# ArnauGabrielAtienza/pytorch_distributed_examples

Hardware: AMD Instinct MI355X
Metric: images/sec (whole node) MNIST DDP + ResNet50 RPC-MP at 1/2/4/8 MI355X (higher is better)
Workload: dtype bf16; 1 GPU; model=mnist_cnn_Net, global_batch=1024, image=1x28x28, parallelism=dp1, hipgraph=True, fused_step=True, rccl_nranks=1, steps_per_graph=5, allreduce=none

## Files before the change

csrc/kernels/cnn_fused.hip:

```cpp
#include <cstddef>
#include <type_traits>

#include "adasum_weights.h"
#include "common.cuh"
#include "optim_device.h"
#include "pde_kernels.h"
#include "xgmi_device.h"

namespace pde {

namespace {

constexpr int T = 1024;
constexpr int NW = T / 64;
constexpr int NI = 4;
constexpr int C1 = 10, C2 = 20, KS = 5, H0 = 28, O1 = 24, P1 = 12, O2 = 8, P2 = 4, F1 = 50, F2 = 10;
constexpr int NX = H0 * H0, NC1 = P1 * P1, NR1 = C1 * NC1, NC2 = P2 * P2, NIN = C2 * NC2;
constexpr int RP16 = 146, RP8 = 148;
static_assert(RP16 >= NC1 && RP8 >= NC1, "channel planes hold the 144 cells");
static_assert(RP16 % 2 == 0 && RP8 % 4 == 0, "P9 reads 4 cells' argmax bytes as one aligned 4-byte word");
constexpr int EP = 148;
constexpr unsigned char AM_DEAD = 0xFF;
constexpr int XP = 36, NXP = H0 * XP;
constexpr int DHP = 52;
constexpr int W1N = C1 * KS * KS, W2N = C2 * C1 * KS * KS, FC1N = F1 * NIN, FC2N = F2 * F1;
constexpr int K2 = C1 * KS * KS;
constexpr int C1P = 16;
constexpr int KS2 = (KS * KS * C1P + 31) / 32;
constexpr int KSW2 = NI * 8 * 8 / 32;
constexpr int CG = 3;
constexpr int NGD = KS * KS * CG;
constexpr int KSD = (NGD + 3) / 4;
constexpr int D2N_P = 24, D2N_RP = 264, D2N_Q = 128;
constexpr int D2N_IM = 7 * D2N_RP + 7 * D2N_P + 2 * D2N_Q + 8;
static_assert(D2N_IM % 8 == 0 && D2N_P % 8 == 0 && D2N_RP % 8 == 0 && D2N_Q % 8 == 0, "d2n: 16-byte slots");
__host__ __device__ constexpr int d2n_ofs(int im, int y, int x, int co) {
  return im * D2N_IM + y * D2N_RP + x * D2N_P + (co >> 3) * D2N_Q + (co & 7);
}
constexpr int D2R = O2 * O2 + 8;
constexpr int MT1 = O1 * O1 / 16;
constexpr int MTD = NC1 * 1 / 16;
constexpr int KSW1 = O1 * O1 / 32;
struct KsRange {
  int lo, hi;
};
__host__ __device__ constexpr bool p7b_tap_live(int cls, int r, int ky, int kx) {
  const int pos = cls * 16 + r, y = pos / P1 - ky, x = pos % P1 - kx;
  return y >= 0 && y < O2 && x >= 0 && x < O2;
}
__host__ __device__ constexpr KsRange p7b_ks_range(int cls) {
  int lo = KSD, hi = 0;
  for (int r = 0; r < 16; ++r)
    for (int ky = 0; ky < KS; ++ky)
      for (int kx = 0; kx < KS; ++kx) {
        if (!p7b_tap_live(cls, r, ky, kx)) continue;
        const int g0 = (ky * KS + kx) * CG, k0 = g0 / 4, k1 = (g0 + CG - 1) / 4;
        lo = k0 < lo ? k0 : lo;
        hi = k1 + 1 > hi ? k1 + 1 : hi;
      }
  return {lo, hi};
}
__host__ __device__ constexpr bool p7b_range_covers(int cls, KsRange q) {
  for (int g = 0; g < NGD; ++g)
    for (int r = 0; r < 16; ++r)
      if (p7b_tap_live(cls, r, g / CG / KS, g / CG % KS) && (g / 4 < q.lo || g / 4 >= q.hi)) return false;
  return q.lo >= 0 && q.hi <= KSD;
}
__host__ __device__ constexpr bool p7b_ranges_ok() {
  int sum = 0;
  for (int c = 0; c < MTD; ++c) {
    if (!p7b_range_covers(c, p7b_ks_range(c))) return false;
    sum += p7b_ks_range(c).hi - p7b_ks_range(c).lo;
  }
  return sum == 126;
}
constexpr bool ks_is(KsRange q, int lo, int hi) { return q.lo == lo && q.hi == hi; }
static_assert(MTD == 9 && NC1 % 16 == 0 && p7b_ranges_ok(), "conv2 dgrad: every live tap inside its class's range");
static_assert(ks_is(p7b_ks_range(0), 0, 7) && ks_is(p7b_ks_range(1), 0, 12) && ks_is(p7b_ks_range(2), 0, 15) &&
                  ks_is(p7b_ks_range(3), 0, KSD) && ks_is(p7b_ks_range(4), 0, KSD) &&
                  ks_is(p7b_ks_range(5), 0, KSD) && ks_is(p7b_ks_range(6), 3, KSD) &&
                  ks_is(p7b_ks_range(7), 7, KSD) && ks_is(p7b_ks_range(8), 12, KSD),
              "conv2 dgrad k-step ranges (rows 0-1, 1-2, 2-3, 4..7, 8-9, 9-10, 10-11)");
__host__ __device__ constexpr uint64_t p7b_pack(bool hi) {
  uint64_t v = 0;
  for (int c = 0; c < MTD; ++c)
    v |= static_cast<uint64_t>(hi ? p7b_ks_range(c).hi : p7b_ks_range(c).lo) << (5 * c);
  return v;
}
constexpr uint64_t P7B_LO = p7b_pack(false), P7B_HI = p7b_pack(true);
static_assert(KSD < 32 && MTD * 5 <= 64, "5-bit fields");
constexpr int P7B_WCLS[NW] = {3, 4, 5, 5, 3, 4, 6, 6, 1, 7, 2, 2, 1, 7, 0, 0};
constexpr int P7B_WPAIR[NW] = {0, 0, 0, 1, 1, 1, 0, 1, 0, 0, 0, 1, 1, 1, 0, 1};
__host__ __device__ constexpr int p7b_wave_steps(int w) {
  const int c = P7B_WCLS[w];
  int n = p7b_ks_range(c).hi - p7b_ks_range(c).lo;
  if (c == 0) n += p7b_ks_range(MTD - 1).hi - p7b_ks_range(MTD - 1).lo;
  return 2 * n;
}
__host__ __device__ constexpr bool p7b_map_ok() {
  for (int c = 0; c < MTD - 1; ++c) {
    int n[2] = {0, 0};
    for (int w = 0; w < NW; ++w)
      if (P7B_WCLS[w] == c) ++n[P7B_WPAIR[w]];
    if (n[0] != 1 || n[1] != 1) return false;
  }
  int tot = 0;
  for (int s = 0; s < 4; ++s) {
    int n = 0;
    for (int w = s; w < NW; w += 4) n += p7b_wave_steps(w);
    if (n < 120 || n > 132) return false;
    tot += n;
  }
  return tot == NI * 126;
}
static_assert(NW == 16 && NI == 4 && p7b_map_ok(), "conv2 dgrad wave map: complete, balanced over the SIMDs");
__host__ __device__ constexpr uint64_t p7b_pack_map(bool pair) {
  uint64_t v = 0;
  for (int w = 0; w < NW; ++w) v |= static_cast<uint64_t>(pair ? P7B_WPAIR[w] : P7B_WCLS[w]) << (4 * w);
  return v;
}
constexpr uint64_t P7B_MCLS = p7b_pack_map(false), P7B_MPAIR = p7b_pack_map(true);
constexpr int O_W1 = 0, O_B1 = O_W1 + W1N, O_W2 = O_B1 + C1, O_B2 = O_W2 + W2N, O_FC1W = O_B2 + C2,
              O_FC1B = O_FC1W + FC1N, O_FC2W = O_FC1B + F1, O_FC2B = O_FC2W + FC2N, NPARAM = O_FC2B + F2;
constexpr int NSLAB = NPARAM - FC1N;
static_assert(O_W2 % 4 == 0 && C2 % 4 == 0 && W2N % 4 == 0, "W2T: float4 columns of 4 co");
constexpr int SLAB_OFS = (32 - O_W2 % 32) % 32;
constexpr int NSLABP = (SLAB_OFS + NSLAB + 31) / 32 * 32;
constexpr int S_FC1B = O_FC1B - FC1N, S_FC2W = O_FC2W - FC1N, S_FC2B = O_FC2B - FC1N;
constexpr int NACT = F1 + NIN;
__host__ __device__ constexpr int act_pitch(int nwg) { return (nwg * NI + 7) & ~7; }
static_assert(O_FC1W % 4 == 0 && FC1N % 4 == 0 && NSLAB % 4 == 0, "float4 slab columns");

__device__ __forceinline__ float hash_u01(unsigned long long seed, unsigned long long id) {
  unsigned long long z = seed + 0x9E3779B97F4A7C15ULL * (id + 1);
  z = (z ^ (z >> 30)) * 0xBF58476D1CE4E5B9ULL;
  z = (z ^ (z >> 27)) * 0x94D049BB133111EBULL;
  z ^= z >> 31;
  return static_cast<float>(z >> 40) * (1.0f / 16777216.0f);
}

__device__ __forceinline__ f32x4 mfma(const u16x8& a, const u16x8& b, const f32x4& c) {
  return __builtin_amdgcn_mfma_f32_16x16x32_bf16(__builtin_bit_cast(bf16x8, a), __builtin_bit_cast(bf16x8, b), c, 0,
                                                 0, 0);
}

template <int CTRL>
__device__ __forceinline__ float dppf(float v) {
  return __builtin_bit_cast(float, __builtin_amdgcn_update_dpp(0, __builtin_bit_cast(int, v), CTRL, 0xF, 0xF, false));
}
__device__ __forceinline__ float lanef(float v, int l) {
  return __builtin_bit_cast(float, __builtin_amdgcn_readlane(__builtin_bit_cast(int, v), l));
}
constexpr int DPP_XOR1 = 0xB1, DPP_XOR2 = 0x4E, DPP_HALF_MIRROR = 0x141, DPP_MIRROR = 0x140;
template <class Op>
__device__ __forceinline__ float wave_all(float v, Op op) {
  v = op(v, dppf<DPP_XOR1>(v));
  v = op(v, dppf<DPP_XOR2>(v));
  v = op(v, dppf<DPP_HALF_MIRROR>(v));
  v = op(v, dppf<DPP_MIRROR>(v));
  return op(op(lanef(v, 0), lanef(v, 16)), op(lanef(v, 32), lanef(v, 48)));
}
__device__ __forceinline__ float wave_sum_dpp(float v) { return wave_all(v, [](float a, float b) { return a + b; }); }
__device__ __forceinline__ float wave_max_dpp(float v) { return wave_all(v, [](float a, float b) { return fmaxf(a, b); }); }

struct CnnSmem {
  alignas(16) uint16_t r1n[NI][NC1][C1P];
  alignas(16) u16x8 w2f[KS2][2][64];
  alignas(16) u16x8 w2d[KSD][64];
  alignas(16) u16x8 w1f[64];
  alignas(16) uint16_t d2n[NI * D2N_IM];
  alignas(16) uint16_t d2[NI][C2][D2R];
  alignas(16) uint16_t zero16[8];
  alignas(8) uint32_t p7tab[KSD * 4][2];
  uint16_t x[NI][NXP];
  uint16_t xpad[18];
  uint16_t x1[NI][NXP];
  uint16_t xonepad[48];
  alignas(16) uint16_t xone[NI][NXP];
  alignas(16) uint16_t r1[NI][C1 * RP16];
  alignas(16) float b1[C1];
  alignas(16) float b2[C2];
  alignas(16) float fc1b[F1];
  alignas(16) float fc2w[FC2N];
  alignas(16) float fc2b[F2];
  alignas(16) float r2[NI][NIN];
  alignas(16) float dp2[NI][NIN];
  float h1[NI][F1], m1[NI][F1], h1d[NI][F1];
  alignas(16) float dh[NI][DHP];
  float mc2[NI][C2];
  float logit[NI][F2], dlog[NI][F2];
  float lossim[NI];
  float valid[NI];
  int label[NI];
  alignas(16) unsigned char a1[NI][C1 * RP8];
  unsigned char a2[NI][NIN];
};
static_assert(sizeof(CnnSmem) <= 160 * 1024, "LDS budget");
static_assert((offsetof(CnnSmem, xone) - offsetof(CnnSmem, x)) / 4 % 32 == 4,
              "xone bank offset from x (P9 B reads: scripts/p9_lds_model.py; x1's: cnn_p1)");
static_assert(offsetof(CnnSmem, w2f) == offsetof(CnnSmem, r1n) + sizeof(uint16_t) * NI * NC1 * C1P &&
                  sizeof(uint32_t) * NI * C1 * EP <= sizeof(uint16_t) * NI * NC1 * C1P + sizeof(u16x8) * KS2 * 2 * 64,
              "e1 aliases r1n + w2f");
static_assert(offsetof(CnnSmem, d2n) == offsetof(CnnSmem, w1f) + sizeof(u16x8) * 64 &&
                  NW * 2 * 64 * sizeof(f32x4) <= sizeof(u16x8) * (KSD * 64 + 64) + sizeof(uint16_t) * NI * D2N_IM,
              "P9 partials alias w2d + w1f + d2n (not e1)");
static_assert(offsetof(CnnSmem, w2d) == offsetof(CnnSmem, w2f) + sizeof(u16x8) * KS2 * 2 * 64, "w2f, w2d adjacent");
constexpr int NT2 = 16 / NW;
constexpr int NFRAG = KS2 * 2 * 64 + KSD * 64 + 64;
constexpr int NF2F = KS2 * 2 * 64, NF2D = KSD * 64;
static_assert(NF2F <= 2 * T && NF2D <= 2 * T && NF2F + NF2D + 64 == NFRAG, "fragment slots");
static_assert(offsetof(CnnSmem, w1f) == offsetof(CnnSmem, w2d) + sizeof(u16x8) * KSD * 64, "w2d, w1f adjacent");
constexpr int FC1_KC = NIN / 32;
constexpr int DP2_JC = 3;
constexpr int DP2_J = 16;
static_assert(F1 - DP2_J * (DP2_JC - 1) <= 20 && DP2_J % 4 == 0 && DHP >= DP2_J * (DP2_JC - 1) + 20, "dp2 chunks");
static_assert(F1 * FC1_KC <= T && NIN * DP2_JC <= T, "fc1 work split");
static_assert(sizeof(float) * NI * NIN * DP2_JC <= sizeof(u16x8) * KS2 * 2 * 64, "dp2 partials alias w2f");
static_assert(NT2 * NW == 16, "conv2 wgrad tiling");

__device__ __forceinline__ void lds_sync() {
  __builtin_amdgcn_fence(__ATOMIC_RELEASE, "workgroup", "local");
  __builtin_amdgcn_s_barrier();
  __builtin_amdgcn_fence(__ATOMIC_ACQUIRE, "workgroup", "local");
}

__device__ __forceinline__ uint32_t lds_addr(const void* p) {
#if defined(__HIP_DEVICE_COMPILE__)
  return (uint32_t)(const __attribute__((address_space(3))) unsigned char*)(p);
#else
  return static_cast<uint32_t>(reinterpret_cast<uintptr_t>(p));
#endif
}
__device__ __forceinline__ u16x8 lds_read16(uint32_t o) {
#if defined(__HIP_DEVICE_COMPILE__)
  return *(const __attribute__((address_space(3))) u16x8*)(o);
#else
  return u16x8{static_cast<uint16_t>(o), 0, 0, 0, 0, 0, 0, 0};
#endif
}

__device__ __forceinline__ void out_st(float* p, float v) {
  asm volatile("global_store_dword %0, %1, off sc1" ::"v"(p), "v"(v) : "memory");
}
__device__ __forceinline__ void out_st_u16x4(uint16_t* p, u16x4 v) { st_vec(reinterpret_cast<u16x4*>(p), v, true); }
__device__ __forceinline__ void out_st4(float* p, f32x4 v) {
  asm volatile("global_store_dwordx4 %0, %1, off sc1" ::"v"(p), "v"(v) : "memory");
}

template <bool TRAIN, class Smem>
__device__ __forceinline__ void cnn_p0(Smem& S, int t, int n0, int B, const float* __restrict__ images,
                                       const int64_t* __restrict__ tgt, const float* __restrict__ params,
                                       const u16x8* __restrict__ frag, const unsigned long long* __restrict__ rng,
                                       float p_drop2, float p_drop1, int training, u16x8 (&fr)[2]) {
  static_assert(NI * NX / 4 <= T, "one image quad per thread");
  constexpr int NH = C1 + C2 + F1 + FC2N + F2;
  static_assert(NH <= T && O_FC2W == O_FC1B + F1 && O_FC2B == O_FC2W + FC2N, "fc1b, fc2w, fc2b contiguous");
  static_assert(offsetof(Smem, fc2b) == offsetof(Smem, fc2w) + sizeof(float) * FC2N, "fc2w, fc2b adjacent");
  static_assert((NI & (NI - 1)) == 0 && 384 % NI == 0, "label threads 384..: slot t & (NI - 1)");
  const int qi = min(t, NI * NX / 4 - 1);
  const int qim = (qi * 4) / NX, qoff = qi * 4 - qim * NX;
  const int hi = min(t, NH - 1);
  const int hsrc = hi < C1 ? O_B1 + hi : hi < C1 + C2 ? O_B2 + hi - C1 : O_FC1B + hi - (C1 + C2);
  const int lslot = t & (NI - 1);
  const int64_t* lbase = tgt != nullptr ? tgt : reinterpret_cast<const int64_t*>(frag);
  const int lidx = tgt != nullptr ? min(n0 + lslot, B - 1) : 0;
  int rofs = 0;
  asm("" : "+v"(rofs));
  const u16x8 fw1 = frag[NF2F + NF2D + (t & 63)];
  const f32x4 img = *reinterpret_cast<const f32x4*>(images + static_cast<long>(min(n0 + qim, B - 1)) * NX + qoff);
  const float hv = params[hsrc];
  unsigned long long r0 = 0;
  if constexpr (TRAIN) r0 = rng[rofs];
  const int lab = reinterpret_cast<const int*>(lbase)[2 * lidx];
  fr[0] = frag[t];
  fr[1] = frag[min(t + T, NF2F - 1)];
  static_assert(H0 % 4 == 0 && XP >= H0 + 6, "image quads within a row; kx = 5 reads stay in the row");
  for (int i = t; i < NI * H0 * (XP - H0 + 1); i += T) {
    const int r = i / (XP - H0 + 1), c = i - r * (XP - H0 + 1);
    if (c > 0) (&S.x[0][0])[r * XP + H0 - 1 + c] = 0;
    (&S.x1[0][0])[r * XP + H0 - 1 + c] = 0;
  }
  if constexpr (TRAIN) {
    constexpr int NZ = (sizeof(Smem::d2n) + sizeof(Smem::d2)) / 16;
    static_assert(offsetof(Smem, d2) == offsetof(Smem, d2n) + sizeof(Smem::d2n) && sizeof(Smem::d2n) % 16 == 0 &&
                      sizeof(Smem::d2) % 16 == 0 && NZ > T && NZ <= 2 * T,
                  "d2n, d2 adjacent: two 16-byte stores per thread");
    static_assert(sizeof(Smem::d2n) == sizeof(uint16_t) * NI * D2N_IM &&
                      d2n_ofs(NI - 1, O2 - 1, O2 - 1, CG * 8 - 1) == NI * D2N_IM - 1 && d2n_ofs(0, 0, 0, 0) == 0,
                  "d2n: the zeroed extent is first to last slot of (image, y, x, co < 24)");
    {
      u16x8* z = reinterpret_cast<u16x8*>(&S.d2n[0]);
      z[t] = u16x8{0, 0, 0, 0, 0, 0, 0, 0};
      if (t + T < NZ) z[t + T] = u16x8{0, 0, 0, 0, 0, 0, 0, 0};
    }
    if (t < 8) S.zero16[t] = 0;
    static_assert((NI * NXP) % 8 == 0 && NI * NXP / 8 <= T, "xone: one 16-byte store per thread");
    if (t < NI * NXP / 8)
      reinterpret_cast<u16x8*>(&S.xone[0][0])[t] =
          u16x8{0x3F80, 0x3F80, 0x3F80, 0x3F80, 0x3F80, 0x3F80, 0x3F80, 0x3F80};
    if (t < KSD * 4) {
      const int g = t, tap = g / CG, cg = g - tap * CG, ky = tap / KS, kx = tap - ky * KS;
      S.p7tab[g][0] = g < NGD ? (static_cast<uint32_t>(ky) << 16) | static_cast<uint32_t>(kx) : 0x80008000u;
      S.p7tab[g][1] = static_cast<uint32_t>(g < NGD ? (-(ky * D2N_RP + kx * D2N_P) + cg * D2N_Q) * 2 : 0);
    }
  }
  if (t < 64) S.w1f[t] = fw1;
  if (t < NI * NX / 4) {
    const int im = qim, off = qoff, n = n0 + im;
    const f32x4 v = n < B ? img : f32x4{0.f, 0.f, 0.f, 0.f};
    const int row = off / H0, col = off - row * H0;
    uint16_t* dst = &S.x[im][row * XP + col];
    const uint16_t b0 = f2bf(v[0]), b1 = f2bf(v[1]), b2 = f2bf(v[2]), b3 = f2bf(v[3]);
    dst[0] = b0; dst[1] = b1; dst[2] = b2; dst[3] = b3;
    uint16_t* d1 = &S.x1[im][row * XP + col];
    if (col > 0) d1[-1] = b0;
    d1[0] = b1; d1[1] = b2; d1[2] = b3;
  }
  if (t < NH) {
    const int hofs = hi < C1             ? static_cast<int>(offsetof(Smem, b1)) + 4 * hi
                     : hi < C1 + C2      ? static_cast<int>(offsetof(Smem, b2)) + 4 * (hi - C1)
                     : hi < C1 + C2 + F1 ? static_cast<int>(offsetof(Smem, fc1b)) + 4 * (hi - (C1 + C2))
                                         : static_cast<int>(offsetof(Smem, fc2w)) + 4 * (hi - (C1 + C2 + F1));
    *reinterpret_cast<float*>(reinterpret_cast<unsigned char*>(&S) + hofs) = hv;
  }
  if constexpr (TRAIN) {
    const unsigned long long seed = r0 * 0xD1B54A32D192ED03ULL;
    const float keep2 = training ? 1.f / (1.f - p_drop2) : 1.f;
    const float keep1 = training ? 1.f / (1.f - p_drop1) : 1.f;
    if (t < NI * C2) {
      const int im = t / C2, c = t - im * C2;
      const unsigned long long id = static_cast<unsigned long long>(n0 + im) * C2 + c;
      S.mc2[im][c] = (!training || hash_u01(seed ^ 0x5bd1e995ULL, id) >= p_drop2) ? keep2 : 0.f;
    } else if (t >= 128 && t < 128 + NI * F1) {
      const int u = t - 128, im = u / F1, j = u - im * F1;
      const unsigned long long id = static_cast<unsigned long long>(n0 + im) * F1 + j;
      S.m1[im][j] = (!training || hash_u01(seed ^ 0x27d4eb2fULL, id) >= p_drop1) ? keep1 : 0.f;
    }
  }
  if (t >= 384 && t < 384 + NI) {
    const bool ok = tgt != nullptr && n0 + lslot < B;
    if constexpr (TRAIN) S.valid[lslot] = ok ? 1.f : 0.f;
    S.label[lslot] = ok ? static_cast<int>(lab) : 0;
  }
}


__device__ __forceinline__ float pool4(const f32x4& v, int& am) {
  am = 0;
  float m = v[0];
  if (v[1] > m) { m = v[1]; am = 1; }
  if (v[2] > m) { m = v[2]; am = 2; }
  if (v[3] > m) { m = v[3]; am = 3; }
  return m;
}

static_assert(P1 % 4 == 0 && MT1 * 4 == NC1, "conv1 tiles: 4 cells of one row");
static_assert((NI * MT1) % NW == 0, "every wave runs the same number of conv1 tiles");
constexpr int NT1 = NI * MT1 / NW;
constexpr int P1_TR = P1 / 4;
static_assert(MT1 % NT1 == 0, "conv1: a wave's tiles lie in one image");
static_assert(NT1 % P1_TR == 0, "conv1: a wave's tiles are whole cell rows");
constexpr int P1_WI = MT1 / NT1;
constexpr int P1_WR = NT1 / P1_TR;
struct P1Tile {
  int im, py, px0;
};
__host__ __device__ constexpr P1Tile p1_tile(int w, int u) {
  return {w / P1_WI, (w % P1_WI) * P1_WR + u / P1_TR, (u % P1_TR) * 4};
}
__host__ __device__ constexpr bool p1_map_ok() {
  for (int tile = 0; tile < NI * MT1; ++tile) {
// ... 243 lines not shown
    fd[1] = frag[NF2F + min(iw + TW, NF2D - 1)];
  }
  constexpr int JPER = F1 - DP2_J * (DP2_JC - 1);
  float w6[JPER];
  {
    const int tc = min(t, NIN * DP2_JC - 1);
    const int jc = tc / NIN, i = tc - jc * NIN;
#pragma unroll
    for (int u = 0; u < JPER; ++u) w6[u] = gFC1W[min(jc * DP2_J + u, F1 - 1) * NIN + i];
  }

  static_assert(NI <= NW, "P4: a wave per image");
  if (wid < NI) {
    const int im = wid, v = lane >> 2, p = lane & 3;
    const bool lv = v < F2;
    const auto [logit, lse, ly, y] = cnn_head(S, S.h1d[im], im, lane);
    const float val = S.valid[im];
    const float dl = (__expf(logit - lse) - (v == y ? 1.f : 0.f)) * val;
    if (lv && p == 0) S.dlog[im][v] = dl;
    if (lane == 0) S.lossim[im] = val * (lse - ly);
    static_assert(F1 <= 64, "P4: a lane per fc1 output");
    const int j = lane < F1 ? lane : 0;
    float sh = 0.f;
#pragma unroll
    for (int vv = 0; vv < F2; ++vv) sh += S.fc2w[vv * F1 + j] * lanef(dl, 4 * vv);
    if (lane < F1) S.dh[im][lane] = (S.h1[im][lane] > 0.f) ? sh * S.m1[im][lane] : 0.f;
  } else {
    static_assert(NC1 % 2 == 0 && RP16 % 2 == 0 && C1 > 8 && C1 <= 10 && C1P == 16 && NI * NC1 <= TW,
                  "r1 from r1n: cell pairs as aligned words, channels 0..7 | 8, 9");
    if (iw < NI * NC1) {
      const uint32_t uw = static_cast<uint32_t>(iw);
      const uint32_t im = uw / NC1, cp = (uw - im * NC1) >> 1, h = uw & 1;
      const uint32_t* src = reinterpret_cast<const uint32_t*>(&S.r1n[0][0][0]) + (uw >> 1) * C1P + h * 4;
      const u32x4 ev = *reinterpret_cast<const u32x4*>(src), od = *reinterpret_cast<const u32x4*>(src + C1P / 2);
      uint32_t* dst = reinterpret_cast<uint32_t*>(&S.r1[im][0]) + h * 8 * (RP16 / 2) + cp;
#pragma unroll
      for (int d = 0; d < 4; ++d)
        if (d == 0 || h == 0) {
          dst[(2 * d) * (RP16 / 2)] = (ev[d] & 0xFFFFu) | (od[d] << 16);
          dst[(2 * d + 1) * (RP16 / 2)] = (ev[d] >> 16) | (od[d] & 0xFFFF0000u);
        }
    }
    u16x8* dst = &S.w2d[0][0];
    dst[iw] = fd[0];
    if (iw + TW < NF2D) dst[iw + TW] = fd[1];
  }
  lds_sync();
  PDE_STAMP(5);
  PDE_STAMP(6);
  PDE_STAMP(7);


  float* dpart = reinterpret_cast<float*>(&S.w2f[0][0][0]);
  {
    const int tc = min(t, NIN * DP2_JC - 1);
    const int jc = tc / NIN, i = tc - jc * NIN;
    const int j0 = jc * DP2_J, nj = jc == DP2_JC - 1 ? F1 - j0 : DP2_J;
    const float* w = w6;
    float s4[NI] = {0.f, 0.f, 0.f, 0.f};
#pragma unroll
    for (int im = 0; im < NI; ++im)
#pragma unroll
      for (int q = 0; q < (JPER + 3) / 4; ++q) {
        const f32x4 d = *reinterpret_cast<const f32x4*>(&S.dh[im][j0 + 4 * q]);
#pragma unroll
        for (int e = 0; e < 4; ++e) {
          const int u = 4 * q + e;
          if (u < JPER) s4[im] += u < nj ? w[u] * d[e] : 0.f;
        }
      }
    if (t < NIN * DP2_JC) {
#pragma unroll
      for (int im = 0; im < NI; ++im) dpart[(jc * NI + im) * NIN + i] = s4[im];
    }
  }
  static_assert(FC2N + F2 <= T, "fc2 weight / bias gradients: one element per thread");
  if (t < FC2N) {
    const int v = t / F1, j = t - v * F1;
    float s = 0.f;
#pragma unroll
    for (int im = 0; im < NI; ++im) s += S.dlog[im][v] * S.h1d[im][j];
    out_st(&slab[S_FC2W + t], s);
  } else if (t < FC2N + F2) {
    const int v = t - FC2N;
    float s = 0.f;
#pragma unroll
    for (int im = 0; im < NI; ++im) s += S.dlog[im][v];
    out_st(&slab[S_FC2B + v], s);
  }
  {
    const int Bk = gridDim.x * NI, Bkp = act_pitch(gridDim.x);
    const bool pad = Bkp != Bk && n0 + NI == Bk;
    for (int row = t; row < NACT; row += T) {
      u16x4 v;
#pragma unroll
      for (int im = 0; im < NI; ++im) v[im] = f2bf(row < F1 ? S.dh[im][row] : S.r2[im][row - F1]);
      out_st_u16x4(acts + static_cast<long>(row) * Bkp + n0, v);
      if (pad) out_st_u16x4(acts + static_cast<long>(row) * Bkp + n0 + NI, u16x4{0, 0, 0, 0});
    }
  }
  if (t < F1) {
    float s = 0.f;
#pragma unroll
    for (int im = 0; im < NI; ++im) s += S.dh[im][t];
    out_st(&slab[S_FC1B + t], s);
  }
  lds_sync();
  constexpr int IH = NI / 2;
  static_assert(NI % 2 == 0 && IH * NIN <= T, "dp2 scatter: two images per thread, one trip");
  if (t < IH * NIN) {
    const int im0 = t / NIN, q = t - im0 * NIN, co = q / NC2, cell = q - co * NC2;
    const int py = cell >> 2, px = cell & 3;
    float pj[2][DP2_JC], rv[2], mk[2];
    int am[2];
#pragma unroll
    for (int u = 0; u < 2; ++u) {
      const int im = im0 + u * IH;
#pragma unroll
      for (int jc = 0; jc < DP2_JC; ++jc) pj[u][jc] = dpart[(jc * NI + im) * NIN + q];
      rv[u] = S.r2[im][q];
      mk[u] = S.mc2[im][co];
      am[u] = S.a2[im][q];
    }
#pragma unroll
    for (int u = 0; u < 2; ++u) {
#pragma unroll
      for (int jc = 0; jc < DP2_JC; ++jc) asm volatile("" : "+v"(pj[u][jc]));
      asm volatile("" : "+v"(rv[u]), "+v"(mk[u]), "+v"(am[u]));
    }
    float v[2];
    uint32_t o2[2], on[2];
#pragma unroll
    for (int u = 0; u < 2; ++u) {
      const int im = im0 + u * IH;
      float s1 = 0.f;
#pragma unroll
      for (int jc = 0; jc < DP2_JC; ++jc) s1 += pj[u][jc];
      v[u] = rv[u] > 0.f ? s1 * mk[u] : 0.f;
      S.dp2[im][q] = v[u];
      const int y = 2 * py + (am[u] >> 1), x = 2 * px + (am[u] & 1);
      o2[u] = static_cast<uint32_t>((im * C2 + co) * D2R + y * O2 + x);
      on[u] = static_cast<uint32_t>(d2n_ofs(im, y, x, co));
    }
#pragma unroll
    for (int u = 0; u < 2; ++u)
      if (rv[u] > 0.f) {
        const uint16_t g = f2bf(v[u]);
        (&S.d2[0][0][0])[o2[u]] = g;
        S.d2n[on[u]] = g;
      }
  }
  lds_sync();
  PDE_STAMP(8);
  if (t >= 448 && t < 448 + C2) {
    const int co = t - 448;
    f32x4 s4 = {0.f, 0.f, 0.f, 0.f};
#pragma unroll
    for (int im = 0; im < NI; ++im)
#pragma unroll
      for (int c = 0; c < NC2; c += 4) s4 += *reinterpret_cast<const f32x4*>(&S.dp2[im][co * NC2 + c]);
    out_st(&slab[O_B2 + co], (s4[0] + s4[1]) + (s4[2] + s4[3]));
  }

  {
    int nb[NT2];
#pragma unroll
    for (int u = 0; u < NT2; ++u) {
      const int kidx = (wid * NT2 + u) * 16 + lr, ci = kidx / 25, r = kidx - ci * 25, ky = r / 5, kx = r - ky * 5;
      nb[u] = kidx < K2 ? ci * RP16 + ky * P1 + kx : 0;
    }
    const uint16_t* arow[2];
#pragma unroll
    for (int mt = 0; mt < 2; ++mt) arow[mt] = &S.d2[0][min(mt * 16 + lr, C2 - 1)][0];
    f32x4 acc[2][NT2];
#pragma unroll
    for (int u = 0; u < NT2; ++u) acc[0][u] = acc[1][u] = f32x4{0.f, 0.f, 0.f, 0.f};
    for (int ks = 0; ks < KSW2; ++ks) {
      const int im = ks >> 1, y = (ks & 1) * 4 + lg;
      u16x8 a[2];
#pragma unroll
      for (int mt = 0; mt < 2; ++mt) a[mt] = *reinterpret_cast<const u16x8*>(arow[mt] + im * C2 * D2R + y * O2);
#pragma unroll
      for (int u = 0; u < NT2; ++u) {
        const int e0 = nb[u] + y * P1;
        const uint32_t* wp = reinterpret_cast<const uint32_t*>(&S.r1[im][0]) + (e0 >> 1);
        const uint32_t sh = static_cast<uint32_t>(e0 & 1) * 2;
        uint32_t w[5];
#pragma unroll
        for (int q = 0; q < 5; ++q) w[q] = wp[q];
        u32x4 v;
#pragma unroll
        for (int q = 0; q < 4; ++q) v[q] = __builtin_amdgcn_alignbyte(w[q + 1], w[q], sh);
        const u16x8 b = __builtin_bit_cast(u16x8, v);
        acc[0][u] = mfma(a[0], b, acc[0][u]);
        acc[1][u] = mfma(a[1], b, acc[1][u]);
      }
    }
#pragma unroll
    for (int mt = 0; mt < 2; ++mt)
#pragma unroll
      for (int u = 0; u < NT2; ++u) {
        const int kidx = (wid * NT2 + u) * 16 + lr, cg = mt * 4 + lg;
        if (cg * 4 < C2 && kidx < K2) out_st4(&slab[O_W2 + (cg * K2 + kidx) * 4], acc[mt][u]);
      }
  }
  PDE_STAMP(9);

  {
    constexpr int MAXT = 2;
    const int cls0 = static_cast<int>(P7B_MCLS >> (4 * wid)) & 15;
    const int im0 = (static_cast<int>(P7B_MPAIR >> (4 * wid)) & 1) * MAXT;
    const int npass = cls0 == 0 ? 2 : 1;
    const uint32_t sbase = lds_addr(smem_raw);
    const uint32_t zpo = sbase + static_cast<uint32_t>(offsetof(CnnSmem, zero16));
    constexpr uint32_t IMB = D2N_IM * 2;
    uint32_t* e1 = reinterpret_cast<uint32_t*>(&S.r1n[0][0][0]);
    auto run_pass = [&](int pass) {
      const int cls = pass == 0 ? cls0 : MTD - 1;
      const int lo = fullk ? 0 : static_cast<int>(P7B_LO >> (5 * cls)) & 31;
      const int hi = fullk ? KSD : static_cast<int>(P7B_HI >> (5 * cls)) & 31;
      const int pos = cls * 16 + lr, ty = pos / P1, tx = pos - ty * P1;
      const u16x2 tyx{static_cast<uint16_t>(tx), static_cast<uint16_t>(ty)};
      const uint32_t tpo = sbase + static_cast<uint32_t>(offsetof(CnnSmem, d2n)) + d2n_ofs(im0, ty, tx, 0) * 2;
      f32x4 acc[MAXT];
#pragma unroll
      for (int u = 0; u < MAXT; ++u) acc[u] = f32x4{0.f, 0.f, 0.f, 0.f};
      const int ci = lr, cell = cls * 16 + lg * 4;
      uint32_t am4[MAXT];
#pragma unroll
      for (int u = 0; u < MAXT; ++u)
        am4[u] = *reinterpret_cast<const uint32_t*>(&S.a1[im0 + u][min(ci, C1 - 1) * RP8 + cell]);

      auto tab = [&](int ks) { return *reinterpret_cast<const u32x2*>(&S.p7tab[min(ks, KSD - 1) * 4 + lg][0]); };
      auto load = [&](const u32x2& e, u16x8 (&a)[MAXT]) {
        const u16x2 kyx = __builtin_bit_cast(u16x2, e[0]);
        const bool ok = (__builtin_bit_cast(uint32_t, static_cast<u16x2>(tyx - kyx)) & 0xFFF8FFF8u) == 0u;
        const uint32_t src = tpo + e[1];
#pragma unroll
        for (int u = 0; u < MAXT; ++u) {
          uint32_t o = ok ? src + u * IMB : zpo;
          asm("" : "+v"(o));
          a[u] = lds_read16(o);
        }
      };
      u16x8 ae[MAXT], ao[MAXT], be, bo;
      load(tab(lo), ae);
      be = S.w2d[lo][lane];
      u32x2 en = tab(lo + 1);
      int ks = lo;
      for (; ks + 2 < hi; ks += 2) {
        u32x2 e = en;
        en = tab(ks + 2);
        load(e, ao);
        bo = S.w2d[ks + 1][lane];
#pragma unroll
        for (int u = 0; u < MAXT; ++u) acc[u] = mfma(ae[u], be, acc[u]);
        e = en;
        en = tab(ks + 3);
        load(e, ae);
        be = S.w2d[ks + 2][lane];
#pragma unroll
        for (int u = 0; u < MAXT; ++u) acc[u] = mfma(ao[u], bo, acc[u]);
      }
      if (ks + 1 < hi) {
        load(en, ao);
        bo = S.w2d[ks + 1][lane];
#pragma unroll
        for (int u = 0; u < MAXT; ++u) acc[u] = mfma(ae[u], be, acc[u]);
#pragma unroll
        for (int u = 0; u < MAXT; ++u) acc[u] = mfma(ao[u], bo, acc[u]);
      } else {
#pragma unroll
        for (int u = 0; u < MAXT; ++u) acc[u] = mfma(ae[u], be, acc[u]);
      }
      if (ci < C1) {
#pragma unroll
        for (int u = 0; u < MAXT; ++u) {
          const int im = im0 + u;
          u32x4 e;
#pragma unroll
          for (int r = 0; r < 4; ++r) {
            const uint32_t am = (am4[u] >> (8 * r)) & 0xFFu;
            e[r] = am == AM_DEAD ? 0u : static_cast<uint32_t>(f2bf(acc[u][r])) << (16 * (am & 1u));
          }
          *reinterpret_cast<u32x4*>(&e1[(im * C1 + ci) * EP + cell]) = e;
        }
      }
    };
    for (int pass = 0; pass < npass; ++pass) run_pass(pass);
  }
  lds_sync();
  PDE_STAMP(10);

  {
    const uint16_t* xw[2];
#pragma unroll
    for (int u = 0; u < 2; ++u) {
      const int k0 = u * 16 + lr, kidx = k0 > 25 ? 17 : k0;
      const int nb = (kidx / 5) * XP + kidx % 5;
      xw[u] = kidx == 25 ? &S.xone[0][0] : ((kidx % 5) & 1 ? &S.x1[0][0] - 1 : &S.x[0][0]) + nb;
    }
    f32x4 acc[2] = {f32x4{0.f, 0.f, 0.f, 0.f}, f32x4{0.f, 0.f, 0.f, 0.f}};
    const int co = lr;
    const int cr = co < C1 ? co : 0;
    const uint32_t* e1 = reinterpret_cast<const uint32_t*>(&S.r1n[0][0][0]);
    constexpr int NK9 = (NI * KSW1 + NW - 1) / NW;
    static_assert(KSW1 * 4 * 2 == NC1 && P1 % 2 == 0, "P9: 4 lane groups x 2 cells per k-step");
    uint32_t m9[NK9];
    u32x2 e9[NK9];
    u16x8 b9[NK9][2];
#pragma unroll
    for (int u9 = 0; u9 < NK9; ++u9) {
      const int ks = wid + u9 * NW;
      if (ks >= NI * KSW1) break;
      const int im = ks / KSW1;
      const uint32_t gi = static_cast<uint32_t>((ks - im * KSW1) * 4 + lg);
      const uint32_t py = (gi * 43u) >> 8, pc = gi - py * 6u;
      const int cell = static_cast<int>(py * P1 + pc * 2);
      m9[u9] = *reinterpret_cast<const uint16_t*>(&S.a1[im][cr * RP8 + cell]);
      e9[u9] = *reinterpret_cast<const u32x2*>(&e1[(im * C1 + cr) * EP + cell]);
      const int off = im * NXP + static_cast<int>(py * 2 * XP + pc * 4);
#pragma unroll
      for (int u = 0; u < 2; ++u) {
        const uint16_t* src = xw[u] + off;
        u32x4 v;
        v[0] = *reinterpret_cast<const uint32_t*>(src);
        v[1] = *reinterpret_cast<const uint32_t*>(src + 2);
        v[2] = *reinterpret_cast<const uint32_t*>(src + XP);
        v[3] = *reinterpret_cast<const uint32_t*>(src + XP + 2);
        b9[u9][u] = __builtin_bit_cast(u16x8, v);
      }
    }
#pragma unroll
    for (int u9 = 0; u9 < NK9; ++u9) {
      if (wid + u9 * NW >= NI * KSW1) break;
      u32x4 a;
#pragma unroll
      for (int c = 0; c < 2; ++c) {
        const bool lower = (m9[u9] >> (8 * c + 1)) & 1u;
        a[c] = lower ? 0u : e9[u9][c];
        a[2 + c] = lower ? e9[u9][c] : 0u;
      }
#pragma unroll
      for (int u = 0; u < 2; ++u) acc[u] = mfma(__builtin_bit_cast(u16x8, a), b9[u9][u], acc[u]);
    }
    f32x4* part = reinterpret_cast<f32x4*>(&S.w2d[0][0]);
    part[(wid * 2 + 0) * 64 + lane] = acc[0];
    part[(wid * 2 + 1) * 64 + lane] = acc[1];
    lds_sync();
    if (stamps != nullptr && t == 0) stamps[blockIdx.x * 16 + 14] = wall_clock64();
    static_assert(O_W1 == 0 && O_B1 == W1N && (W1N + C1) % 4 == 0, "conv1 gradients: one float4 run");
    if (wid * 64 < W1N + C1) {
      const bool live = t < W1N + C1;
      const int c = t < W1N ? t / 25 : (live ? t - W1N : 0);
      const int kidx = t < W1N ? t - c * 25 : 25;
      const int u = kidx >> 4;
      const int l = (c >> 2) * 16 + (kidx & 15), r = c & 3;
      float s = 0.f;
#pragma unroll
      for (int w = 0; w < NW; ++w) s += part[(w * 2 + u) * 64 + l][r];
      const int si = __builtin_bit_cast(int, s);
      const f32x4 q{s, __builtin_bit_cast(float, __builtin_amdgcn_update_dpp(0, si, 0x55, 0xF, 0xF, false)),
                    __builtin_bit_cast(float, __builtin_amdgcn_update_dpp(0, si, 0xAA, 0xF, 0xF, false)),
                    __builtin_bit_cast(float, __builtin_amdgcn_update_dpp(0, si, 0xFF, 0xF, 0xF, false))};
      if (live && (t & 3) == 0) out_st4(&slab[O_W1 + t], q);
    }
  }
  PDE_STAMP(11);

  if (wid == 0) {
    const float l = wave_sum_dpp(lane < NI ? S.lossim[lane] : 0.f);
    if (lane == 0) out_st(&loss_part[blockIdx.x], l);
  }
  if (stamps != nullptr) {
    asm volatile("s_waitcnt vmcnt(0)" ::: "memory");
    __syncthreads();
    PDE_STAMP(12);
  }
}

__global__ __launch_bounds__(256) void k_cnn_prep(const float* __restrict__ params, u16x8* __restrict__ frag) {
  const int e = blockIdx.x * 256 + threadIdx.x;
  if (e >= NFRAG) return;
  const float* gW1 = params + O_W1;
  const float* gW2 = params + O_W2;
  u16x8 f;
  if (e < KS2 * 2 * 64) {
    const int ks = e >> 7, nt = (e >> 6) & 1, l = e & 63;
    const int co = nt * 16 + (l & 15), g = l >> 4, tap = 2 * ks + (g >> 1), c8 = (g & 1) * 8;
#pragma unroll
    for (int j = 0; j < 8; ++j)
      f[j] = (co < C2 && tap < KS * KS && c8 + j < C1) ? f2bf(gW2[co * K2 + (c8 + j) * KS * KS + tap]) : 0;
  } else if (e < KS2 * 2 * 64 + KSD * 64) {
    const int e2 = e - KS2 * 2 * 64, ks = e2 >> 6, l = e2 & 63;
    const int ci = l & 15, g = ks * 4 + (l >> 4), tap = g / CG, c0 = (g - tap * CG) * 8;
#pragma unroll
    for (int j = 0; j < 8; ++j)
      f[j] = (g < NGD && ci < C1 && c0 + j < C2) ? f2bf(gW2[(c0 + j) * K2 + ci * 25 + tap]) : 0;
  } else {
    const int l = e - KS2 * 2 * 64 - KSD * 64;
    const int co = l & 15, k0 = (l >> 4) * 8;
#pragma unroll
    for (int j = 0; j < 8; ++j) {
      const int k = k0 + j, ky = k / 6, kx = k - ky * 6;
      f[j] = (co < C1 && k < KS * 6 && kx < KS) ? f2bf(gW1[co * 25 + ky * KS + kx]) : 0;
    }
  }
  frag[e] = f;
}

__device__ __forceinline__ void write_frag(uint16_t* __restrict__ f, int p, float w) {
  const uint16_t b = f2bf(w);
  if (p >= O_W2 && p < O_W2 + W2N) {
    const int q = p - O_W2, co = q / K2, r = q - co * K2, ci = r / (KS * KS), tap = r - ci * (KS * KS);
    const int g = ((tap & 1) << 1) | (ci >> 3);
    const int e = ((tap >> 1) << 7) | ((co >> 4) << 6) | (g << 4) | (co & 15);
    f[e * 8 + (ci & 7)] = b;
    const int gd = tap * CG + (co >> 3);
    const int e2 = KS2 * 2 * 64 + (gd >> 2) * 64 + (((gd & 3) << 4) | ci);
    f[e2 * 8 + (co & 7)] = b;
  } else if (p >= O_W1 && p < O_W1 + W1N) {
    const int co = p / (KS * KS), k25 = p - co * (KS * KS);
    const int k = (k25 / KS) * 6 + k25 % KS;
    const int e = KS2 * 2 * 64 + KSD * 64 + (((k >> 3) << 4) | co);
    f[e * 8 + (k & 7)] = b;
  }
}

__global__ __launch_bounds__(256) void k_cnn_sgd(float* __restrict__ params, const float* __restrict__ grads,
                                                 const float* __restrict__ hp, uint16_t* __restrict__ frag,
                                                 int* __restrict__ step) {
  if (step != nullptr && blockIdx.x == 0 && threadIdx.x == 0) step[0] += 1;
  const int p = blockIdx.x * 256 + threadIdx.x;
  if (p >= NPARAM) return;
  const float w = params[p] - hp[HP_LR] * (grads[p] * hp[HP_GRAD_SCALE]);
  params[p] = w;
  write_frag(frag, p, w);
}

constexpr int RED_COLS = 16;
constexpr int RED_T = 512, RED_LANES = RED_T / RED_COLS;
constexpr int NSLAB4 = NSLAB / 4;
constexpr int RED_SLAB_BLOCKS = (NSLAB4 + RED_COLS - 1) / RED_COLS;
// ... 767 lines not shown
```

Measured before the change: 42.75 million images/s.

## Split conv2 wgrad and dgrad across disjoint wave groups to run concurrently

```diff
diff --git a/csrc/kernels/cnn_fused.hip b/csrc/kernels/cnn_fused.hip
--- a/csrc/kernels/cnn_fused.hip
+++ b/csrc/kernels/cnn_fused.hip
@@ -89,37 +89,59 @@
 }
 constexpr uint64_t P7B_LO = p7b_pack(false), P7B_HI = p7b_pack(true);
 static_assert(KSD < 32 && MTD * 5 <= 64, "5-bit fields");
-constexpr int P7B_WCLS[NW] = {3, 4, 5, 5, 3, 4, 6, 6, 1, 7, 2, 2, 1, 7, 0, 0};
-constexpr int P7B_WPAIR[NW] = {0, 0, 0, 1, 1, 1, 0, 1, 0, 0, 0, 1, 1, 1, 0, 1};
+constexpr int P7_DW = 8;
+constexpr int P7B_WCLS[P7_DW] = {3, 4, 5, 6, 1, 7, 0, 2};
+constexpr int NT2 = 16 / (NW - P7_DW);
+__host__ __device__ constexpr int p7a_tile(int w, int u) { return (w - P7_DW) * NT2 + u; }
 __host__ __device__ constexpr int p7b_wave_steps(int w) {
   const int c = P7B_WCLS[w];
   int n = p7b_ks_range(c).hi - p7b_ks_range(c).lo;
   if (c == 0) n += p7b_ks_range(MTD - 1).hi - p7b_ks_range(MTD - 1).lo;
-  return 2 * n;
+  return n;
 }
 __host__ __device__ constexpr bool p7b_map_ok() {
-  for (int c = 0; c < MTD - 1; ++c) {
-    int n[2] = {0, 0};
-    for (int w = 0; w < NW; ++w)
-      if (P7B_WCLS[w] == c) ++n[P7B_WPAIR[w]];
-    if (n[0] != 1 || n[1] != 1) return false;
-  }
+  for (int c = 0; c < MTD; ++c)
+    for (int im = 0; im < NI; ++im) {
+      int n = 0;
+      for (int w = 0; w < P7_DW; ++w)
+        if (P7B_WCLS[w] == (c == MTD - 1 ? 0 : c)) ++n;
+      if (n != 1) return false;
+    }
   int tot = 0;
   for (int s = 0; s < 4; ++s) {
-    int n = 0;
-    for (int w = s; w < NW; w += 4) n += p7b_wave_steps(w);
-    if (n < 120 || n > 132) return false;
+    int n = 0, nd = 0, nw = 0;
+    for (int w = s; w < NW; w += 4) {
+      if (w < P7_DW) {
+        n += p7b_wave_steps(w);
+        ++nd;
+      } else {
+        ++nw;
+      }
+    }
+    if (n < 31 || n > 33 || nd != 2 || nw != 2) return false;
     tot += n;
   }
-  return tot == NI * 126;
+  return tot == 126;
+}
+__host__ __device__ constexpr bool p7a_map_ok() {
+  for (int nt = 0; nt < 16; ++nt)
+    for (int mt = 0; mt < 2; ++mt) {
+      int n = 0;
+      for (int w = P7_DW; w < NW; ++w)
+        for (int u = 0; u < NT2; ++u)
+          if (p7a_tile(w, u) == nt) ++n;
+      if (n != 1) return false;
+    }
+  return true;
 }
 static_assert(NW == 16 && NI == 4 && p7b_map_ok(), "conv2 dgrad wave map: complete, balanced over the SIMDs");
-__host__ __device__ constexpr uint64_t p7b_pack_map(bool pair) {
+static_assert(NT2 == 2 && NT2 * (NW - P7_DW) == 16 && p7a_map_ok(), "conv2 wgrad wave map: complete");
+__host__ __device__ constexpr uint64_t p7b_pack_map() {
   uint64_t v = 0;
-  for (int w = 0; w < NW; ++w) v |= static_cast<uint64_t>(pair ? P7B_WPAIR[w] : P7B_WCLS[w]) << (4 * w);
+  for (int w = 0; w < P7_DW; ++w) v |= static_cast<uint64_t>(P7B_WCLS[w]) << (4 * w);
   return v;
 }
-constexpr uint64_t P7B_MCLS = p7b_pack_map(false), P7B_MPAIR = p7b_pack_map(true);
+constexpr uint64_t P7B_MCLS = p7b_pack_map();
 constexpr int O_W1 = 0, O_B1 = O_W1 + W1N, O_W2 = O_B1 + C1, O_B2 = O_W2 + W2N, O_FC1W = O_B2 + C2,
               O_FC1B = O_FC1W + FC1N, O_FC2W = O_FC1B + F1, O_FC2B = O_FC2W + FC2N, NPARAM = O_FC2B + F2;
 constexpr int NSLAB = NPARAM - FC1N;
@@ -205,7 +227,6 @@
                   NW * 2 * 64 * sizeof(f32x4) <= sizeof(u16x8) * (KSD * 64 + 64) + sizeof(uint16_t) * NI * D2N_IM,
               "P9 partials alias w2d + w1f + d2n (not e1)");
 static_assert(offsetof(CnnSmem, w2d) == offsetof(CnnSmem, w2f) + sizeof(u16x8) * KS2 * 2 * 64, "w2f, w2d adjacent");
-constexpr int NT2 = 16 / NW;
 constexpr int NFRAG = KS2 * 2 * 64 + KSD * 64 + 64;
 constexpr int NF2F = KS2 * 2 * 64, NF2D = KSD * 64;
 static_assert(NF2F <= 2 * T && NF2D <= 2 * T && NF2F + NF2D + 64 == NFRAG, "fragment slots");
@@ -216,7 +237,6 @@
 static_assert(F1 - DP2_J * (DP2_JC - 1) <= 20 && DP2_J % 4 == 0 && DHP >= DP2_J * (DP2_JC - 1) + 20, "dp2 chunks");
 static_assert(F1 * FC1_KC <= T && NIN * DP2_JC <= T, "fc1 work split");
 static_assert(sizeof(float) * NI * NIN * DP2_JC <= sizeof(u16x8) * KS2 * 2 * 64, "dp2 partials alias w2f");
-static_assert(NT2 * NW == 16, "conv2 wgrad tiling");
 
 __device__ __forceinline__ void lds_sync() {
   __builtin_amdgcn_fence(__ATOMIC_RELEASE, "workgroup", "local");
@@ -766,21 +786,23 @@
   }
   lds_sync();
   PDE_STAMP(8);
-  if (t >= 448 && t < 448 + C2) {
-    const int co = t - 448;
-    f32x4 s4 = {0.f, 0.f, 0.f, 0.f};
-#pragma unroll
-    for (int im = 0; im < NI; ++im)
-#pragma unroll
-      for (int c = 0; c < NC2; c += 4) s4 += *reinterpret_cast<const f32x4*>(&S.dp2[im][co * NC2 + c]);
-    out_st(&slab[O_B2 + co], (s4[0] + s4[1]) + (s4[2] + s4[3]));
-  }
-
-  {
+  if (wid >= P7_DW) {
+    __builtin_amdgcn_s_setprio(3);
+    constexpr int TB2 = (NW - 1) * 64;
+    static_assert(C2 <= 64 && NW - 1 >= P7_DW, "conv2 bias gradient on a wgrad wave");
+    if (t >= TB2 && t < TB2 + C2) {
+      const int co = t - TB2;
+      f32x4 s4 = {0.f, 0.f, 0.f, 0.f};
+#pragma unroll
+      for (int im = 0; im < NI; ++im)
+#pragma unroll
+        for (int c = 0; c < NC2; c += 4) s4 += *reinterpret_cast<const f32x4*>(&S.dp2[im][co * NC2 + c]);
+      out_st(&slab[O_B2 + co], (s4[0] + s4[1]) + (s4[2] + s4[3]));
+    }
     int nb[NT2];
 #pragma unroll
     for (int u = 0; u < NT2; ++u) {
-      const int kidx = (wid * NT2 + u) * 16 + lr, ci = kidx / 25, r = kidx - ci * 25, ky = r / 5, kx = r - ky * 5;
+      const int kidx = p7a_tile(wid, u) * 16 + lr, ci = kidx / 25, r = kidx - ci * 25, ky = r / 5, kx = r - ky * 5;
       nb[u] = kidx < K2 ? ci * RP16 + ky * P1 + kx : 0;
     }
     const uint16_t* arow[2];
@@ -814,16 +836,14 @@
     for (int mt = 0; mt < 2; ++mt)
 #pragma unroll
       for (int u = 0; u < NT2; ++u) {
-        const int kidx = (wid * NT2 + u) * 16 + lr, cg = mt * 4 + lg;
+        const int kidx = p7a_tile(wid, u) * 16 + lr, cg = mt * 4 + lg;
         if (cg * 4 < C2 && kidx < K2) out_st4(&slab[O_W2 + (cg * K2 + kidx) * 4], acc[mt][u]);
       }
-  }
-  PDE_STAMP(9);
-
-  {
-    constexpr int MAXT = 2;
+    __builtin_amdgcn_s_setprio(0);
+  } else {
+    constexpr int MAXT = NI;
     const int cls0 = static_cast<int>(P7B_MCLS >> (4 * wid)) & 15;
-    const int im0 = (static_cast<int>(P7B_MPAIR >> (4 * wid)) & 1) * MAXT;
+    constexpr int im0 = 0;
     const int npass = cls0 == 0 ? 2 : 1;
     const uint32_t sbase = lds_addr(smem_raw);
     const uint32_t zpo = sbase + static_cast<uint32_t>(offsetof(CnnSmem, zero16));
@@ -903,6 +923,7 @@
     };
     for (int pass = 0; pass < npass; ++pass) run_pass(pass);
   }
+  PDE_STAMP(9);
   lds_sync();
   PDE_STAMP(10);
 
```

After: 44.19 million images/s (median of 6 runs). +3.4%, better.
